# OFA-Sys/ONE-PEACE

Measured on NVIDIA H100. Metric: encoder_samples_per_sec, higher is better.
Workload: dtype bf16

## Files before the change

### one_peace_b200/csrc/gemm_wgmma.cu

```cuda
#include "common.cuh"
#include "gemm.h"

#include <mutex>

namespace opb {

constexpr int kBlockM = 128;
constexpr int kBlockN = 256;
constexpr int kBlockK = 64;
constexpr int kStages = 4;
constexpr int kABytes = kBlockM * kBlockK * 2;
constexpr int kBBytes = kBlockN * kBlockK * 2;
constexpr int kStageBytes = kABytes + kBBytes;
constexpr int kThreads = 384;
constexpr int kBandM = 8;
constexpr int kResidBatch = 16;

struct EpiOperands {
  float2 row[kBlockM];
  float colsum[kBlockN], bias[kBlockN], gamma[kBlockN], colscale[kBlockN];
};
constexpr int kStagerThreads = 96;
constexpr int kSmemBytes = kStages * kStageBytes + 1024 + 2 * sizeof(EpiOperands) + 1024;

struct GemmGeom {
  int M, N, K;
  int kb_inner;
  int num_k_blocks;
  int groups;
  int a_group_c0;
  int b_group_rows;
  int a_mn;
  int b_mn;
  int kb_per_piece;
  int m_pad;
  float* split_ws;
};

OPB_DEVICE void fence_acc(float (&d)[128]) {
#pragma unroll
  for (int i = 0; i < 128; ++i) asm volatile("" : "+f"(d[i])::"memory");
}

template <int TA, int TB>
OPB_DEVICE void wgmma_m64n256k16(float (&d)[128], uint64_t desc_a, uint64_t desc_b, uint32_t scale_d) {
  asm volatile(
      "{\n\t"
      ".reg .pred p;\n\t"
      "setp.ne.b32 p, %130, 0;\n\t"
      "wgmma.mma_async.sync.aligned.m64n256k16.f32.bf16.bf16 "
      "{"
      "%0, %1, %2, %3, %4, %5, %6, %7, %8, %9, %10, %11, %12, %13, %14, %15, "
      "%16, %17, %18, %19, %20, %21, %22, %23, %24, %25, %26, %27, %28, %29, %30, %31, "
      "%32, %33, %34, %35, %36, %37, %38, %39, %40, %41, %42, %43, %44, %45, %46, %47, "
      "%48, %49, %50, %51, %52, %53, %54, %55, %56, %57, %58, %59, %60, %61, %62, %63, "
      "%64, %65, %66, %67, %68, %69, %70, %71, %72, %73, %74, %75, %76, %77, %78, %79, "
      "%80, %81, %82, %83, %84, %85, %86, %87, %88, %89, %90, %91, %92, %93, %94, %95, "
      "%96, %97, %98, %99, %100, %101, %102, %103, %104, %105, %106, %107, %108, %109, %110, %111, "
      "%112, %113, %114, %115, %116, %117, %118, %119, %120, %121, %122, %123, %124, %125, %126, %127"
      "}, %128, %129, p, 1, 1, %131, %132;\n\t"
      "}\n"
      : "+f"(d[0]), "+f"(d[1]), "+f"(d[2]), "+f"(d[3]), "+f"(d[4]), "+f"(d[5]), "+f"(d[6]), "+f"(d[7]),
        "+f"(d[8]), "+f"(d[9]), "+f"(d[10]), "+f"(d[11]), "+f"(d[12]), "+f"(d[13]), "+f"(d[14]), "+f"(d[15]),
        "+f"(d[16]), "+f"(d[17]), "+f"(d[18]), "+f"(d[19]), "+f"(d[20]), "+f"(d[21]), "+f"(d[22]), "+f"(d[23]),
        "+f"(d[24]), "+f"(d[25]), "+f"(d[26]), "+f"(d[27]), "+f"(d[28]), "+f"(d[29]), "+f"(d[30]), "+f"(d[31]),
        "+f"(d[32]), "+f"(d[33]), "+f"(d[34]), "+f"(d[35]), "+f"(d[36]), "+f"(d[37]), "+f"(d[38]), "+f"(d[39]),
        "+f"(d[40]), "+f"(d[41]), "+f"(d[42]), "+f"(d[43]), "+f"(d[44]), "+f"(d[45]), "+f"(d[46]), "+f"(d[47]),
        "+f"(d[48]), "+f"(d[49]), "+f"(d[50]), "+f"(d[51]), "+f"(d[52]), "+f"(d[53]), "+f"(d[54]), "+f"(d[55]),
        "+f"(d[56]), "+f"(d[57]), "+f"(d[58]), "+f"(d[59]), "+f"(d[60]), "+f"(d[61]), "+f"(d[62]), "+f"(d[63]),
        "+f"(d[64]), "+f"(d[65]), "+f"(d[66]), "+f"(d[67]), "+f"(d[68]), "+f"(d[69]), "+f"(d[70]), "+f"(d[71]),
        "+f"(d[72]), "+f"(d[73]), "+f"(d[74]), "+f"(d[75]), "+f"(d[76]), "+f"(d[77]), "+f"(d[78]), "+f"(d[79]),
        "+f"(d[80]), "+f"(d[81]), "+f"(d[82]), "+f"(d[83]), "+f"(d[84]), "+f"(d[85]), "+f"(d[86]), "+f"(d[87]),
        "+f"(d[88]), "+f"(d[89]), "+f"(d[90]), "+f"(d[91]), "+f"(d[92]), "+f"(d[93]), "+f"(d[94]), "+f"(d[95]),
        "+f"(d[96]), "+f"(d[97]), "+f"(d[98]), "+f"(d[99]), "+f"(d[100]), "+f"(d[101]), "+f"(d[102]), "+f"(d[103]),
        "+f"(d[104]), "+f"(d[105]), "+f"(d[106]), "+f"(d[107]), "+f"(d[108]), "+f"(d[109]), "+f"(d[110]), "+f"(d[111]),
        "+f"(d[112]), "+f"(d[113]), "+f"(d[114]), "+f"(d[115]), "+f"(d[116]), "+f"(d[117]), "+f"(d[118]), "+f"(d[119]),
        "+f"(d[120]), "+f"(d[121]), "+f"(d[122]), "+f"(d[123]), "+f"(d[124]), "+f"(d[125]), "+f"(d[126]), "+f"(d[127])
      : "l"(desc_a), "l"(desc_b), "r"(scale_d), "n"(TA), "n"(TB));
}

template <bool kFusedVar = false>
OPB_DEVICE void load_ln_stats(const GemmEpilogue& ep, int row, int M, float& mu, float& rs) {
  mu = 0.f; rs = 1.f;
  const int rc = row < M ? row : M - 1;
  if (ep.ln_partial != nullptr) {
    float s1 = 0.f, s2 = 0.f;
#pragma unroll 8
    for (int p = 0; p < ep.ln_parts; ++p) {
      const float2 v = *reinterpret_cast<const float2*>(ep.ln_partial + (static_cast<long>(p) * M + rc) * 2);
      s1 += v.x; s2 += v.y;
    }
    mu = s1 / ep.ln_dim;
    const float ex2 = s2 / ep.ln_dim;
    const float var = kFusedVar ? fmaf(-mu, mu, ex2) : __fsub_rn(ex2, __fmul_rn(mu, mu));
    rs = rsqrtf(fmaxf(var, 0.f) + ep.ln_eps);
  } else if (ep.ln_mu != nullptr) {
    mu = ep.ln_mu[rc];
    rs = ep.ln_rstd[rc];
  }
}

OPB_DEVICE float2 ldf2(const float* p) { return *reinterpret_cast<const float2*>(p); }
OPB_DEVICE float quad_sum(float v) {
  v += __shfl_xor_sync(0xffffffffu, v, 1);
  return v + __shfl_xor_sync(0xffffffffu, v, 2);
}

template <int TA, int TB>
OPB_DEVICE void mainloop(float (&d)[128], uint8_t* smem, uint64_t* full, uint64_t* empty, int num_k_blocks, int cw,
                         uint32_t it0) {
  constexpr uint32_t step_a = TA ? 2048 : 32, step_b = TB ? 2048 : 32;
  const bool signal = (threadIdx.x & 31) == 0;
  for (int kb = 0; kb < num_k_blocks; ++kb) {
    const uint32_t it = it0 + kb;
    const uint32_t s = it % kStages;
    mbar_wait_quiet(&full[s], (it / kStages) & 1);
    const uint32_t sa = smem_u32(smem + s * kStageBytes) + cw * 8192;
    const uint32_t sb = smem_u32(smem + s * kStageBytes + kABytes);
    fence_acc(d);
    wgmma_fence();
#pragma unroll
    for (int k = 0; k < kBlockK / 16; ++k)
      wgmma_m64n256k16<TA, TB>(d, wgmma_desc_sw128(sa + k * step_a, 8192), wgmma_desc_sw128(sb + k * step_b, 8192),
                               (kb > 0 || k > 0) ? 1u : 0u);
    wgmma_commit();
    fence_acc(d);
    if (kb > 0) {
      wgmma_wait<1>();
      fence_acc(d);
      __syncwarp();
      if (signal) mbar_arrive(&empty[(it - 1) % kStages]);
    }
  }
  wgmma_wait<0>();
  fence_acc(d);
  __syncwarp();
  if (signal) mbar_arrive(&empty[(it0 + num_k_blocks - 1) % kStages]);
}

constexpr bool epi_staged(int epi) { return epi != EPI_LSE_PARTIAL && epi != EPI_SOFTMAX_GRAD; }

template <int EPI>
OPB_DEVICE void stage_epi_operands(EpiOperands* st, const GemmEpilogue& ep, const GemmGeom& geo, int m_blk, int n_blk, int grp,
                                   int t) {
  if (ep.ln_partial != nullptr || ep.ln_mu != nullptr) {
    for (int r = t; r < kBlockM; r += kStagerThreads) {
      float mu, rs;
      load_ln_stats<EPI == EPI_GEGLU_BF16 || EPI == EPI_RESID_F32>(ep, m_blk * kBlockM + r, geo.M, mu, rs);
      st->row[r] = make_float2(mu, rs);
    }
  }
  for (int c = t; c < kBlockN; c += kStagerThreads) {
    const int tc = n_blk * kBlockN + c;
    const bool ok = tc < geo.N;
    const int col = grp * geo.N + tc;
    st->colsum[c] = ok && ep.ln_colsum != nullptr ? ep.ln_colsum[col] : 0.f;
    st->bias[c] = ok && ep.bias != nullptr ? ep.bias[col] : 0.f;
    st->gamma[c] = ok && ep.gamma != nullptr ? ep.gamma[col] : 0.f;
    st->colscale[c] = ok && ep.colscale != nullptr ? ep.colscale[col] : 0.f;
  }
}

template <int EPI>
OPB_DEVICE void epilogue(const float (&d)[128], const GemmEpilogue& ep, const GemmGeom& geo, const EpiOperands* st, int m_blk,
                         int n_blk, int grp, int cw) {
  const int M = geo.M, N = geo.N;
  const int t = threadIdx.x & 127;
  const int lane = t & 31;
  const int quad = lane & 3;
  const int rloc = cw * 64 + (t >> 5) * 16 + (lane >> 2);
  const int rbase = m_blk * kBlockM + rloc;
  const int col0 = n_blk * kBlockN;
  const int gcol0 = grp * N;
#pragma unroll
  for (int h = 0; h < 2; ++h) {
    const int row = rbase + 8 * h;
    bool row_ok = row < M;
    if (ep.out_group > 0 && ep.out_group_valid > 0 && (row % ep.out_group) >= ep.out_group_valid) row_ok = false;
    long out_row = row;
    if (ep.out_group > 0) out_row = static_cast<long>(row / ep.out_group) * ep.out_group_stride + (row % ep.out_group) + ep.out_row_offset;
    long res_row = out_row;
    if (ep.resid_period > 0) res_row = (row % ep.resid_period) + ep.resid_row_offset;

    if constexpr (EPI == EPI_LSE_PARTIAL) {
      const float scale = *ep.scale_ptr;
      const int tgt = row + ep.target_offset;
      const int nv = ep.n_valid > 0 ? ep.n_valid : N;
      float m = -INFINITY;
#pragma unroll
      for (int j = 0; j < 32; ++j) {
        const int col = col0 + 8 * j + 2 * quad;
        if (col < nv) m = fmaxf(m, scale * d[4 * j + 2 * h]);
        if (col + 1 < nv) m = fmaxf(m, scale * d[4 * j + 2 * h + 1]);
      }
      float ssum = 0.f, zsum = 0.f, best = -INFINITY, ztgt = 0.f;
      int best_idx = 0, has_tgt = 0;
#pragma unroll
      for (int j = 0; j < 32; ++j) {
#pragma unroll
        for (int e = 0; e < 2; ++e) {
          const int col = col0 + 8 * j + 2 * quad + e;
          if (col < nv) {
            const float z = scale * d[4 * j + 2 * h + e];
            ssum += __expf(z - m);
            zsum += z;
            if (z > best) { best = z; best_idx = col; }
            if (col == tgt) { ztgt = z; has_tgt = 1; }
          }
        }
      }
#pragma unroll
      for (int o = 1; o <= 2; o <<= 1) {
        const float m2 = __shfl_xor_sync(0xffffffffu, m, o), s2 = __shfl_xor_sync(0xffffffffu, ssum, o);
        const float zs2 = __shfl_xor_sync(0xffffffffu, zsum, o), b2 = __shfl_xor_sync(0xffffffffu, best, o);
        const int i2 = __shfl_xor_sync(0xffffffffu, best_idx, o), h2 = __shfl_xor_sync(0xffffffffu, has_tgt, o);
        const float zt2 = __shfl_xor_sync(0xffffffffu, ztgt, o);
        const float mn = fmaxf(m, m2);
        ssum = (m > -INFINITY ? ssum * __expf(m - mn) : 0.f) + (m2 > -INFINITY ? s2 * __expf(m2 - mn) : 0.f);
        m = mn;
        zsum += zs2;
        if (b2 > best || (b2 == best && i2 < best_idx)) { best = b2; best_idx = i2; }
        if (h2) { ztgt = zt2; has_tgt = 1; }
      }
      if (row_ok && quad == 0) {
        float* w = ep.ws + (static_cast<long>(n_blk) * M + row) * 8;
        *reinterpret_cast<float4*>(w) = make_float4(m, ssum, zsum, best);
        *reinterpret_cast<float4*>(w + 4) = make_float4(__int_as_float(best_idx), ztgt, has_tgt ? 1.f : 0.f, 0.f);
      }
    } else if constexpr (EPI == EPI_SOFTMAX_GRAD) {
      const float scale = *ep.scale_ptr;
      const float gscale = scale * ep.coef;
      const int tgt = row + ep.target_offset;
      const float lse = row_ok ? ep.row_lse[row] : 0.f;
      const float hit = 1.f - ep.eps - ep.eps_i;
      const int nv = ep.n_valid > 0 ? ep.n_valid : N;
      float gz = 0.f;
#pragma unroll
      for (int j = 0; j < 32; ++j) {
        const int col = col0 + 8 * j + 2 * quad;
        if (!row_ok || col >= N) continue;
        float gq[2];
#pragma unroll
        for (int e = 0; e < 2; ++e) {
          const float z = scale * d[4 * j + 2 * h + e];
          float g = __expf(z - lse) - ep.eps_i;
          if (col + e == tgt) g -= hit;
          if (col + e >= nv) g = 0.f;
          gz += g * z;
          gq[e] = g * gscale;
        }
        *reinterpret_cast<uint32_t*>(reinterpret_cast<__nv_bfloat16*>(ep.out) + out_row * ep.ldo + col) = pack_bf16x2(gq[0], gq[1]);
      }
      gz = quad_sum(gz);
      if (row_ok && quad == 0) ep.ws[static_cast<long>(n_blk) * M + row] = gz;
    } else {
      const float2 mr = (ep.ln_partial != nullptr || ep.ln_mu != nullptr) ? st->row[rloc + 8 * h] : make_float2(0.f, 1.f);
      const float mu = mr.x, rs = mr.y;
      const bool has_ln = ep.ln_colsum != nullptr;
      float st_sum = 0.f, st_sq = 0.f;
      if constexpr (EPI == EPI_GEGLU_BF16) {
        __nv_bfloat16* out = reinterpret_cast<__nv_bfloat16*>(ep.out) + out_row * ep.ldo + n_blk * (kBlockN / 2);
#pragma unroll
        for (int j = 0; j < 16; ++j) {
          const int tc = 8 * j + 2 * quad;
          float g0 = d[4 * j + 2 * h], g1 = d[4 * j + 2 * h + 1];
          float l0 = d[4 * (j + 16) + 2 * h], l1 = d[4 * (j + 16) + 2 * h + 1];
          if (has_ln) {
            const float2 cg = ldf2(st->colsum + tc), cl = ldf2(st->colsum + tc + kBlockN / 2);
            g0 = rs * (g0 - mu * cg.x); g1 = rs * (g1 - mu * cg.y);
            l0 = rs * (l0 - mu * cl.x); l1 = rs * (l1 - mu * cl.y);
          }
          if (ep.bias != nullptr) {
            const float2 bg = ldf2(st->bias + tc), bl = ldf2(st->bias + tc + kBlockN / 2);
            g0 += bg.x; g1 += bg.y; l0 += bl.x; l1 += bl.y;
          }
          const float u0 = gelu_erf(g0) * l0, u1 = gelu_erf(g1) * l1;
          st_sum += u0 + u1;
          st_sq += u0 * u0 + u1 * u1;
          if (row_ok) *reinterpret_cast<uint32_t*>(out + tc) = pack_bf16x2(u0, u1);
        }
        st_sum = quad_sum(st_sum);
        st_sq = quad_sum(st_sq);
        if (row_ok && quad == 0 && ep.stats_out != nullptr) {
          *reinterpret_cast<float2*>(ep.stats_out + (static_cast<long>(n_blk * 2) * M + row) * 2) = make_float2(st_sum, st_sq);
          *reinterpret_cast<float2*>(ep.stats_out + (static_cast<long>(n_blk * 2 + 1) * M + row) * 2) = make_float2(0.f, 0.f);
        }
      } else {
#pragma unroll
        for (int jb = 0; jb < 32; jb += kResidBatch) {
          float2 res[kResidBatch];
          if constexpr (EPI == EPI_RESID_F32) {
            if (ep.resid != nullptr && row_ok) {
              const float* rp = ep.resid + res_row * ep.ldr + gcol0;
#pragma unroll
              for (int jj = 0; jj < kResidBatch; ++jj) {
                const int tc = col0 + 8 * (jb + jj) + 2 * quad;
                if (tc < N) res[jj] = ldf2(rp + tc);
              }
            }
          }
#pragma unroll
          for (int jj = 0; jj < kResidBatch; ++jj) {
            const int j = jb + jj;
            const int lc = 8 * j + 2 * quad;
            const int tc = col0 + lc;
            if (tc >= N) continue;
            const int col = gcol0 + tc;
            float x0 = d[4 * j + 2 * h], x1 = d[4 * j + 2 * h + 1];
            if (has_ln) {
              const float2 c = ldf2(st->colsum + lc);
              x0 = rs * (x0 - mu * c.x); x1 = rs * (x1 - mu * c.y);
            }
            if (ep.bias != nullptr) {
              const float2 b = ldf2(st->bias + lc);
              x0 += b.x; x1 += b.y;
            }
            if constexpr (EPI == EPI_STORE_BF16 || EPI == EPI_GELU_BF16) {
              if (ep.colscale != nullptr) {
                const float2 s = ldf2(st->colscale + lc);
                x0 *= s.x; x1 *= s.y;
              }
              if constexpr (EPI == EPI_GELU_BF16) { x0 = gelu_erf(x0); x1 = gelu_erf(x1); }
              if (row_ok) *reinterpret_cast<uint32_t*>(reinterpret_cast<__nv_bfloat16*>(ep.out) + out_row * ep.ldo + col) = pack_bf16x2(x0, x1);
            } else {
              if constexpr (EPI == EPI_RESID_F32) {
                if (ep.gamma != nullptr) {
                  const float2 g = ldf2(st->gamma + lc);
                  x0 *= g.x; x1 *= g.y;
                }
                if (ep.resid != nullptr && row_ok) {
                  x0 += res[jj].x; x1 += res[jj].y;
                }
                st_sum += x0 + x1;
                st_sq += x0 * x0 + x1 * x1;
                if (row_ok && ep.out_bf16 != nullptr)
                  *reinterpret_cast<uint32_t*>(reinterpret_cast<__nv_bfloat16*>(ep.out_bf16) + out_row * ep.ldo_bf16 + col) = pack_bf16x2(x0, x1);
              }
              if (row_ok) *reinterpret_cast<float2*>(reinterpret_cast<float*>(ep.out) + out_row * ep.ldo + col) = make_float2(x0, x1);
            }
          }
        }
        if constexpr (EPI == EPI_RESID_F32) {
          st_sum = quad_sum(st_sum);
          st_sq = quad_sum(st_sq);
          if (row_ok && quad == 0 && ep.stats_out != nullptr)
            *reinterpret_cast<float2*>(ep.stats_out + (static_cast<long>(n_blk) * M + row) * 2) = make_float2(st_sum, st_sq);
        }
      }
    }
  }
}

struct TileCoord {
  int piece, grp, m_blk, n_blk;
};
OPB_DEVICE TileCoord tile_coord(int unit, int num_m_tiles, int num_n_tiles, int groups) {
  const int per_group = num_m_tiles * num_n_tiles;
  TileCoord c;
  c.piece = unit / (per_group * groups);
  const int tile = unit - c.piece * per_group * groups;
  c.grp = tile / per_group;
  const int tin = tile - c.grp * per_group;
  const int band = tin / (kBandM * num_n_tiles);
  const int m0 = band * kBandM;
  const int band_rows = min(kBandM, num_m_tiles - m0);
  const int r = tin - m0 * num_n_tiles;
  c.m_blk = m0 + r % band_rows;
  c.n_blk = r / band_rows;
  return c;
}

template <int EPI>
__global__ void __launch_bounds__(kThreads, 1)
gemm_bf16_kernel(const __grid_constant__ CUtensorMap tm_a, const __grid_constant__ CUtensorMap tm_b, const GemmEpilogue ep,
                 const GemmGeom geo) {
  extern __shared__ __align__(1024) uint8_t smem_raw[];
  uint8_t* smem = smem_raw;
  if ((smem_u32(smem) & 1023u) != 0) __trap();
  uint64_t* full = reinterpret_cast<uint64_t*>(smem + kStages * kStageBytes);
  uint64_t* empty = full + kStages;
  uint64_t* epi_full = empty + kStages;
  uint64_t* epi_empty = epi_full + 2;
  EpiOperands* epi_ops = reinterpret_cast<EpiOperands*>(smem + kStages * kStageBytes + 1024);

  const int wg = threadIdx.x >> 7;
  const int num_m_tiles = (geo.M + kBlockM - 1) / kBlockM;
  const int num_n_tiles = (geo.N + kBlockN - 1) / kBlockN;
  const int pieces = geo.kb_per_piece > 0 ? (geo.num_k_blocks + geo.kb_per_piece - 1) / geo.kb_per_piece : 1;
  const int units = num_m_tiles * num_n_tiles * geo.groups * pieces;
  const bool staged = epi_staged(EPI) && geo.kb_per_piece == 0;

  if (threadIdx.x == 0) {
    tma_prefetch_desc(&tm_a);
    tma_prefetch_desc(&tm_b);
    for (int i = 0; i < kStages; ++i) {
      mbar_init(&full[i], 1);
      mbar_init(&empty[i], 8);
    }
    for (int i = 0; i < 2; ++i) {
      mbar_init(&epi_full[i], kStagerThreads);
      mbar_init(&epi_empty[i], 8);
    }
    fence_barrier_init();
  }
  __syncthreads();

  if (wg == 0) {
    asm volatile("setmaxnreg.dec.sync.aligned.u32 40;");
    if (threadIdx.x == 0) {
      uint32_t it = 0;
      for (int unit = blockIdx.x; unit < units; unit += gridDim.x) {
        const TileCoord tc = tile_coord(unit, num_m_tiles, num_n_tiles, geo.groups);
        const int kb0 = geo.kb_per_piece > 0 ? tc.piece * geo.kb_per_piece : 0;
        const int kb1 = geo.kb_per_piece > 0 ? min(geo.num_k_blocks, kb0 + geo.kb_per_piece) : geo.num_k_blocks;
        const int a_row = tc.m_blk * kBlockM;
        const int b_row = tc.grp * geo.b_group_rows + tc.n_blk * kBlockN;
        const int a_c0 = tc.grp * geo.a_group_c0;
        int kin = kb0 % geo.kb_inner, tap = kb0 / geo.kb_inner;
        for (int kb = kb0; kb < kb1; ++kb, ++it) {
          const uint32_t s = it % kStages;
          mbar_wait_quiet(&empty[s], ((it / kStages) & 1) ^ 1);
          uint8_t* sa = smem + s * kStageBytes;
          uint8_t* sb = sa + kABytes;
          mbar_arrive_expect_tx(&full[s], kStageBytes);
          if (geo.a_mn) {
#pragma unroll
            for (int i = 0; i < kBlockM / 64; ++i) tma_load_2d(&tm_a, &full[s], sa + i * 8192, a_row + 64 * i, kb * kBlockK);
          } else {
            tma_load_3d(&tm_a, &full[s], sa, a_c0 + kin * kBlockK, tap, a_row);
          }
          if (geo.b_mn) {
#pragma unroll
            for (int i = 0; i < kBlockN / 64; ++i) tma_load_2d(&tm_b, &full[s], sb + i * 8192, b_row + 64 * i, kb * kBlockK);
          } else {
            tma_load_2d(&tm_b, &full[s], sb, kb * kBlockK, b_row);
          }
          if (++kin == geo.kb_inner) { kin = 0; ++tap; }
        }
      }
    } else if (threadIdx.x >= 32 && staged) {
      uint32_t j = 0;
      for (int unit = blockIdx.x; unit < units; unit += gridDim.x, ++j) {
        const TileCoord tc = tile_coord(unit, num_m_tiles, num_n_tiles, geo.groups);
        mbar_wait_quiet(&epi_empty[j & 1], ((j >> 1) & 1) ^ 1);
        stage_epi_operands<EPI>(&epi_ops[j & 1], ep, geo, tc.m_blk, tc.n_blk, tc.grp, threadIdx.x - 32);
        mbar_arrive(&epi_full[j & 1]);
      }
    }
  } else {
    asm volatile("setmaxnreg.inc.sync.aligned.u32 232;");
    const int cw = wg - 1;
    float d[128];
#pragma unroll
    for (int i = 0; i < 128; ++i) d[i] = 0.f;
    uint32_t it = 0, j = 0;
    for (int unit = blockIdx.x; unit < units; unit += gridDim.x, ++j) {
      const TileCoord tc = tile_coord(unit, num_m_tiles, num_n_tiles, geo.groups);
      const int kb0 = geo.kb_per_piece > 0 ? tc.piece * geo.kb_per_piece : 0;
      const int kb1 = geo.kb_per_piece > 0 ? min(geo.num_k_blocks, kb0 + geo.kb_per_piece) : geo.num_k_blocks;
      if (geo.a_mn) {
        if (geo.b_mn) mainloop<1, 1>(d, smem, full, empty, kb1 - kb0, cw, it);
        else mainloop<1, 0>(d, smem, full, empty, kb1 - kb0, cw, it);
      } else {
        if (geo.b_mn) mainloop<0, 1>(d, smem, full, empty, kb1 - kb0, cw, it);
        else mainloop<0, 0>(d, smem, full, empty, kb1 - kb0, cw, it);
      }
      it += kb1 - kb0;
      if (geo.kb_per_piece > 0) {
        const int t = threadIdx.x & 127, lane = t & 31;
        const int r0 = tc.m_blk * kBlockM + cw * 64 + (t >> 5) * 16 + (lane >> 2);
        float* w = geo.split_ws + static_cast<long>(tc.piece) * geo.m_pad * geo.N;
#pragma unroll
        for (int h = 0; h < 2; ++h) {
#pragma unroll
          for (int c = 0; c < 32; ++c) {
            const int col = tc.n_blk * kBlockN + 8 * c + 2 * (lane & 3);
            if (col < geo.N)
              *reinterpret_cast<float2*>(w + static_cast<long>(r0 + 8 * h) * geo.N + col) = make_float2(d[4 * c + 2 * h], d[4 * c + 2 * h + 1]);
          }
        }
      } else if (staged) {
        mbar_wait_quiet(&epi_full[j & 1], (j >> 1) & 1);
        epilogue<EPI>(d, ep, geo, &epi_ops[j & 1], tc.m_blk, tc.n_blk, tc.grp, cw);
        __syncwarp();
        if ((threadIdx.x & 31) == 0) mbar_arrive(&epi_empty[j & 1]);
      } else {
        epilogue<EPI>(d, ep, geo, nullptr, tc.m_blk, tc.n_blk, tc.grp, cw);
      }
    }
  }
}

__global__ void __launch_bounds__(256)
gemm_split_epilogue_kernel(const GemmEpilogue ep, const GemmGeom geo, int pieces, int epi) {
  __shared__ float red[2][8];
  const int M = geo.M, N = geo.N;
  const int row = blockIdx.x;
  float mu, rs;
  if (ep.ln_partial != nullptr) {
    float s1 = 0.f, s2 = 0.f;
    for (int p = threadIdx.x; p < ep.ln_parts; p += blockDim.x) {
      const float2 v = *reinterpret_cast<const float2*>(ep.ln_partial + (static_cast<long>(p) * M + row) * 2);
      s1 += v.x; s2 += v.y;
    }
    s1 = warp_sum(s1); s2 = warp_sum(s2);
    if ((threadIdx.x & 31) == 0) { red[0][threadIdx.x >> 5] = s1; red[1][threadIdx.x >> 5] = s2; }
    __syncthreads();
    s1 = s2 = 0.f;
    for (int i = 0; i < 8; ++i) { s1 += red[0][i]; s2 += red[1][i]; }
    mu = s1 / ep.ln_dim;
    rs = rsqrtf(fmaxf(s2 / ep.ln_dim - mu * mu, 0.f) + ep.ln_eps);
  } else {
    load_ln_stats(ep, row, M, mu, rs);
  }
  const int t = blockIdx.y;
  const int col = t * kBlockN + threadIdx.x;
  const long slab = static_cast<long>(geo.m_pad) * N;
  float x = 0.f;
  if (col < N) {
    const float* w = geo.split_ws + static_cast<long>(row) * N + col;
    for (int p = 0; p < pieces; ++p) x += w[p * slab];
    if (ep.ln_colsum) x = rs * (x - mu * ep.ln_colsum[col]);
    if (ep.bias) x += ep.bias[col];
    if (epi == EPI_STORE_BF16) {
      if (ep.colscale) x *= ep.colscale[col];
      reinterpret_cast<__nv_bfloat16*>(ep.out)[static_cast<long>(row) * ep.ldo + col] = __float2bfloat16(x);
    } else {
      if (ep.gamma) x *= ep.gamma[col];
      if (ep.resid) x += ep.resid[static_cast<long>(row) * ep.ldr + col];
      reinterpret_cast<float*>(ep.out)[static_cast<long>(row) * ep.ldo + col] = x;
      if (ep.out_bf16) reinterpret_cast<__nv_bfloat16*>(ep.out_bf16)[static_cast<long>(row) * ep.ldo_bf16 + col] = __float2bfloat16(x);
    }
  }
  if (ep.stats_out != nullptr) {
    const float s1 = warp_sum(x), s2 = warp_sum(x * x);
    __syncthreads();
    if ((threadIdx.x & 31) == 0) { red[0][threadIdx.x >> 5] = s1; red[1][threadIdx.x >> 5] = s2; }
    __syncthreads();
    if (threadIdx.x == 0) {
      float a = 0.f, b = 0.f;
      for (int i = 0; i < 8; ++i) { a += red[0][i]; b += red[1][i]; }
      *reinterpret_cast<float2*>(ep.stats_out + (static_cast<long>(t) * M + row) * 2) = make_float2(a, b);
    }
  }
}

typedef CUresult (*PFN_encodeTiled)(CUtensorMap*, CUtensorMapDataType, cuuint32_t, void*, const cuuint64_t*,
                                    const cuuint64_t*, const cuuint32_t*, const cuuint32_t*, CUtensorMapInterleave,
                                    CUtensorMapSwizzle, CUtensorMapL2promotion, CUtensorMapFloatOOBfill);

static PFN_encodeTiled get_encode_fn() {
  static PFN_encodeTiled fn = nullptr;
  static std::once_flag once;
  std::call_once(once, [] {
    void* p = nullptr;
    cudaDriverEntryPointQueryResult qres;
    if (cudaGetDriverEntryPoint("cuTensorMapEncodeTiled", &p, cudaEnableDefault, &qres) == cudaSuccess &&
        qres == cudaDriverEntryPointSuccess) {
      fn = reinterpret_cast<PFN_encodeTiled>(p);
    }
  });
  return fn;
}

int make_tmap_bf16_2d(CUtensorMap* out, const void* ptr, uint64_t rows, uint64_t cols, uint64_t ld,
                      uint32_t box_rows) {
  PFN_encodeTiled enc = get_encode_fn();
  if (enc == nullptr) return OPB_ERR_CUDA;
  if ((reinterpret_cast<uintptr_t>(ptr) & 15) != 0 || (ld * 2) % 16 != 0) return OPB_ERR_INVALID;
  cuuint64_t gdim[2] = {cols, rows};
  cuuint64_t gstride[1] = {ld * 2};
  cuuint32_t box[2] = {static_cast<cuuint32_t>(kBlockK), box_rows};
  cuuint32_t estr[2] = {1, 1};
  CUresult r = enc(out, CU_TENSOR_MAP_DATA_TYPE_BFLOAT16, 2, const_cast<void*>(ptr), gdim, gstride, box, estr,
                   CU_TENSOR_MAP_INTERLEAVE_NONE, CU_TENSOR_MAP_SWIZZLE_128B, CU_TENSOR_MAP_L2_PROMOTION_L2_256B,
                   CU_TENSOR_MAP_FLOAT_OOB_FILL_NONE);
  return r == CUDA_SUCCESS ? OPB_OK : OPB_ERR_CUDA;
}

int make_tmap_bf16_3d(CUtensorMap* out, const void* ptr, uint64_t k_inner, uint64_t taps, uint64_t tap_stride,
                      uint64_t rows, uint64_t row_stride, uint32_t box_rows) {
  PFN_encodeTiled enc = get_encode_fn();
  if (enc == nullptr) return OPB_ERR_CUDA;
  if ((reinterpret_cast<uintptr_t>(ptr) & 15) != 0 || (tap_stride * 2) % 16 != 0 || (row_stride * 2) % 16 != 0)
    return OPB_ERR_INVALID;
  cuuint64_t gdim[3] = {k_inner, taps, rows};
  cuuint64_t gstride[2] = {tap_stride * 2, row_stride * 2};
  cuuint32_t box[3] = {static_cast<cuuint32_t>(kBlockK), 1, box_rows};
  cuuint32_t estr[3] = {1, 1, 1};
  CUresult r = enc(out, CU_TENSOR_MAP_DATA_TYPE_BFLOAT16, 3, const_cast<void*>(ptr), gdim, gstride, box, estr,
                   CU_TENSOR_MAP_INTERLEAVE_NONE, CU_TENSOR_MAP_SWIZZLE_128B, CU_TENSOR_MAP_L2_PROMOTION_L2_256B,
                   CU_TENSOR_MAP_FLOAT_OOB_FILL_NONE);
  return r == CUDA_SUCCESS ? OPB_OK : OPB_ERR_CUDA;
}

int make_tmap_bf16_batched(CUtensorMap* out, const void* ptr, uint64_t cols, uint64_t rows, uint64_t ld, uint64_t batches,
                           uint64_t batch_stride, uint32_t box_rows) {
  PFN_encodeTiled enc = get_encode_fn();
  if (enc == nullptr) return OPB_ERR_CUDA;
  if ((reinterpret_cast<uintptr_t>(ptr) & 15) != 0 || (ld * 2) % 16 != 0 || (batch_stride * 2) % 16 != 0)
    return OPB_ERR_INVALID;
  cuuint64_t gdim[3] = {cols, rows, batches};
  cuuint64_t gstride[2] = {ld * 2, batch_stride * 2};
  cuuint32_t box[3] = {static_cast<cuuint32_t>(kBlockK), box_rows, 1};
  cuuint32_t estr[3] = {1, 1, 1};
  CUresult r = enc(out, CU_TENSOR_MAP_DATA_TYPE_BFLOAT16, 3, const_cast<void*>(ptr), gdim, gstride, box, estr,
                   CU_TENSOR_MAP_INTERLEAVE_NONE, CU_TENSOR_MAP_SWIZZLE_128B, CU_TENSOR_MAP_L2_PROMOTION_L2_256B,
                   CU_TENSOR_MAP_FLOAT_OOB_FILL_NONE);
  return r == CUDA_SUCCESS ? OPB_OK : OPB_ERR_CUDA;
}

template <int EPI>
static int launch_gemm(const CUtensorMap& ta, const CUtensorMap& tb, const GemmEpilogue& ep, const GemmGeom& geo,
                       cudaStream_t stream) {
  auto kern = gemm_bf16_kernel<EPI>;
  static int resident = 0;
  if (resident == 0) {
    if (cudaFuncSetAttribute(kern, cudaFuncAttributeMaxDynamicSharedMemorySize, kSmemBytes) != cudaSuccess)
      return OPB_ERR_CUDA;
    int per_sm = 0;
    if (cudaOccupancyMaxActiveBlocksPerMultiprocessor(&per_sm, kern, kThreads, kSmemBytes) != cudaSuccess || per_sm < 1)
      return OPB_ERR_CUDA;
    resident = per_sm * sm_count();
  }
  const int pieces = geo.kb_per_piece > 0 ? (geo.num_k_blocks + geo.kb_per_piece - 1) / geo.kb_per_piece : 1;
  const long units = static_cast<long>((geo.M + kBlockM - 1) / kBlockM) * ((geo.N + kBlockN - 1) / kBlockN) * geo.groups * pieces;
  const unsigned grid = static_cast<unsigned>(units < resident ? units : resident);
  kern<<<grid, kThreads, kSmemBytes, stream>>>(ta, tb, ep, geo);
  return cudaGetLastError() == cudaSuccess ? OPB_OK : OPB_ERR_CUDA;
}

static int dispatch_gemm(int epi, const CUtensorMap& ta, const CUtensorMap& tb, const GemmEpilogue& ep, const GemmGeom& geo,
                         cudaStream_t stream) {
  switch (epi) {
    case EPI_STORE_BF16: return launch_gemm<EPI_STORE_BF16>(ta, tb, ep, geo, stream);
    case EPI_GELU_BF16: return launch_gemm<EPI_GELU_BF16>(ta, tb, ep, geo, stream);
    case EPI_GEGLU_BF16: return launch_gemm<EPI_GEGLU_BF16>(ta, tb, ep, geo, stream);
    case EPI_RESID_F32: return launch_gemm<EPI_RESID_F32>(ta, tb, ep, geo, stream);
    case EPI_STORE_F32: return launch_gemm<EPI_STORE_F32>(ta, tb, ep, geo, stream);
    case EPI_LSE_PARTIAL: return launch_gemm<EPI_LSE_PARTIAL>(ta, tb, ep, geo, stream);
    case EPI_SOFTMAX_GRAD: return launch_gemm<EPI_SOFTMAX_GRAD>(ta, tb, ep, geo, stream);
    default: return OPB_ERR_INVALID;
  }
}

struct ByteSpan {
  const char* begin;
  const char* end;
};
static ByteSpan row_span(const void* p, long lo, long hi, long ld, long cols, int esz) {
  const char* c = static_cast<const char*>(p);
  return {c + lo * ld * esz, c + (hi * ld + cols) * esz};
}
static bool spans_meet(const ByteSpan& a, const ByteSpan& b) { return a.begin < b.end && b.begin < a.end; }

static bool resid_aliasing_ok(const GemmEpilogue& ep, int M, long cols) {
  if (ep.resid == nullptr) return true;
  auto out_row = [&](long m) {
    return ep.out_group > 0 ? (m / ep.out_group) * ep.out_group_stride + m % ep.out_group + ep.out_row_offset : m;
  };
  const long g = ep.out_group > 0 ? ep.out_group : M, last = M - 1, q = last / g;
  const long corners[5] = {0, (g < M ? g : M) - 1, q * g, last, q > 0 ? q * g - 1 : 0};
  long lo = out_row(0), hi = lo;
  for (long m : corners) {
    lo = out_row(m) < lo ? out_row(m) : lo;
    hi = out_row(m) > hi ? out_row(m) : hi;
  }
  long rlo = lo, rhi = hi;
  if (ep.resid_period > 0) {
    rlo = ep.resid_row_offset;
    rhi = rlo + (ep.resid_period < M ? ep.resid_period : M) - 1;
  }
  const ByteSpan res = row_span(ep.resid, rlo, rhi, ep.ldr, cols, 4);
  if (ep.out_bf16 != nullptr && spans_meet(res, row_span(ep.out_bf16, lo, hi, ep.ldo_bf16, cols, 2))) return false;
  if (!spans_meet(res, row_span(ep.out, lo, hi, ep.ldo, cols, 4))) return true;
  return ep.resid == ep.out && ep.ldr == ep.ldo && ep.resid_period == 0;
}

static GemmGeom plain_geom(int M, int N, int K) {
  GemmGeom geo;
  geo.M = M; geo.N = N; geo.K = K;
  geo.num_k_blocks = (K + kBlockK - 1) / kBlockK;
  geo.kb_inner = geo.num_k_blocks;
  geo.groups = 1;
  geo.a_group_c0 = 0;
  geo.b_group_rows = 0;
  geo.a_mn = geo.b_mn = 0;
  geo.kb_per_piece = 0;
  geo.m_pad = 0;
  geo.split_ws = nullptr;
  return geo;
}

int gemm_bf16(const void* A, int lda, const void* B, int ldb, int M, int N, int K, int epi, const GemmEpilogue& ep,
              int cta_group, cudaStream_t stream) {
  if (M <= 0 || N <= 0 || K <= 0) return OPB_ERR_INVALID;
  if (K % 8 != 0 || N % 8 != 0 || lda % 8 != 0 || ldb % 8 != 0) return OPB_ERR_INVALID;
  if (epi == EPI_GEGLU_BF16 && N % kBlockN != 0) return OPB_ERR_INVALID;
  if (cta_group < 0 || cta_group > 2) return OPB_ERR_INVALID;
  if (epi == EPI_RESID_F32 && !resid_aliasing_ok(ep, M, N)) return OPB_ERR_INVALID;
  GemmGeom geo = plain_geom(M, N, K);
  const int m_tiles = (M + kBlockM - 1) / kBlockM, n_tiles = (N + kBlockN - 1) / kBlockN;
  const bool split_ok = (epi == EPI_RESID_F32 || (epi == EPI_STORE_BF16 && ep.stats_out == nullptr)) && ep.workspace != nullptr &&
                        ep.out_group == 0 && ep.resid_period == 0 && M <= 2 * kBlockM && geo.num_k_blocks >= 8;
  int pieces = 1;
  if (split_ok) {
    const long slab_bytes = static_cast<long>(m_tiles) * kBlockM * N * 4;
    pieces = sm_count() / (m_tiles * n_tiles);
    if (pieces > geo.num_k_blocks / 2) pieces = geo.num_k_blocks / 2;
    if (pieces > ep.workspace_bytes / slab_bytes) pieces = static_cast<int>(ep.workspace_bytes / slab_bytes);
    if (pieces >= 2) {
      geo.kb_per_piece = (geo.num_k_blocks + pieces - 1) / pieces;
      pieces = (geo.num_k_blocks + geo.kb_per_piece - 1) / geo.kb_per_piece;
      geo.m_pad = m_tiles * kBlockM;
      geo.split_ws = reinterpret_cast<float*>(ep.workspace);
    }
  }
  CUtensorMap ta, tb;
  int rc = make_tmap_bf16_3d(&ta, A, K, 1, lda, M, lda, kBlockM);
  if (rc != OPB_OK) return rc;
  rc = make_tmap_bf16_2d(&tb, B, N, K, ldb, kBlockN);
  if (rc != OPB_OK) return rc;
  rc = dispatch_gemm(epi, ta, tb, ep, geo, stream);
  if (rc != OPB_OK || geo.kb_per_piece == 0) return rc;
  gemm_split_epilogue_kernel<<<dim3(M, n_tiles), 256, 0, stream>>>(ep, geo, pieces, epi);
  return cudaGetLastError() == cudaSuccess ? OPB_OK : OPB_ERR_CUDA;
}

int gemm_bf16_t(const void* A, int lda, int a_mn, const void* B, int ldb, int b_mn, int M, int N, int K, int epi,
                const GemmEpilogue& ep, int cta_group, cudaStream_t stream) {
  if (M <= 0 || N <= 0 || K <= 0 || lda % 8 != 0 || ldb % 8 != 0 || N % 8 != 0) return OPB_ERR_INVALID;
  if (epi != EPI_STORE_BF16 && epi != EPI_STORE_F32) return OPB_ERR_INVALID;
  if ((!a_mn && K % 8 != 0) || (!b_mn && K % 8 != 0) || (a_mn && M % 8 != 0)) return OPB_ERR_INVALID;
  if (cta_group < 0 || cta_group > 2) return OPB_ERR_INVALID;
  GemmGeom geo = plain_geom(M, N, K);
  geo.a_mn = a_mn ? 1 : 0;
  geo.b_mn = b_mn ? 1 : 0;
  CUtensorMap ta, tb;
  int rc = a_mn ? make_tmap_bf16_2d(&ta, A, K, M, lda, 64) : make_tmap_bf16_3d(&ta, A, K, 1, lda, M, lda, kBlockM);
  if (rc != OPB_OK) return rc;
  rc = b_mn ? make_tmap_bf16_2d(&tb, B, K, N, ldb, 64) : make_tmap_bf16_2d(&tb, B, N, K, ldb, kBlockN);
  if (rc != OPB_OK) return rc;
  return dispatch_gemm(epi, ta, tb, ep, geo, stream);
}

int gemm_bf16_grouped_window(const void* X, const void* W, int rows, int groups, int c_pad, int taps, int n_per_group,
                             int epi, const GemmEpilogue& ep, cudaStream_t stream) {
  if (rows <= 0 || groups <= 0 || taps <= 0 || n_per_group <= 0) return OPB_ERR_INVALID;
  if (c_pad % kBlockK != 0 || n_per_group % 8 != 0 || n_per_group > kBlockN) return OPB_ERR_INVALID;
  if (epi == EPI_GEGLU_BF16 || epi == EPI_LSE_PARTIAL || epi == EPI_SOFTMAX_GRAD) return OPB_ERR_INVALID;
  if (epi == EPI_RESID_F32 && !resid_aliasing_ok(ep, rows, static_cast<long>(groups) * n_per_group)) return OPB_ERR_INVALID;
  GemmGeom geo = plain_geom(rows, n_per_group, taps * c_pad);
  geo.kb_inner = c_pad / kBlockK;
  geo.num_k_blocks = taps * geo.kb_inner;
  geo.groups = groups;
  geo.a_group_c0 = c_pad;
  geo.b_group_rows = n_per_group;
  const long row_stride = static_cast<long>(groups) * c_pad;
  CUtensorMap ta, tb;
  int rc = make_tmap_bf16_3d(&ta, X, row_stride, taps, row_stride, rows, row_stride, kBlockM);
  if (rc != OPB_OK) return rc;
  rc = make_tmap_bf16_2d(&tb, W, static_cast<uint64_t>(groups) * n_per_group, geo.K, geo.K, kBlockN);
  if (rc != OPB_OK) return rc;
  return dispatch_gemm(epi, ta, tb, ep, geo, stream);
}

}
```

Baseline: 756.0.

## Split last partial wave of GEMM tiles across CTAs by consumer half

When the tile count leaves a partial final wave of at most half the grid, each remaining tile becomes two units. In each unit only one consumer warpgroup computes its 64-row half and runs the epilogue, while the other just drains the pipeline barriers. This spreads the tail across more SMs so each one issues half the tensor-core work, shortening the last wave. In exchange, the producer still loads full A and B tiles for both halves, which doubles the tail's memory traffic.

```diff
diff --git a/one_peace_b200/csrc/gemm_wgmma.cu b/one_peace_b200/csrc/gemm_wgmma.cu
--- a/one_peace_b200/csrc/gemm_wgmma.cu
+++ b/one_peace_b200/csrc/gemm_wgmma.cu
@@ -370,6 +370,37 @@
   return c;
 }
 
+struct UnitMap {
+  int whole;
+  int units;
+  OPB_DEVICE int tile(int unit, int& half) const {
+    if (unit < whole) {
+      half = -1;
+      return unit;
+    }
+    half = (unit - whole) & 1;
+    return whole + ((unit - whole) >> 1);
+  }
+};
+OPB_DEVICE UnitMap unit_map(int tiles, int grid, bool split_last_round) {
+  const int whole = tiles - tiles % grid, rem = tiles - whole;
+  UnitMap m{tiles, tiles};
+  if (split_last_round && whole > 0 && rem > 0 && 2 * rem <= grid) {
+    m.whole = whole;
+    m.units = whole + 2 * rem;
+  }
+  return m;
+}
+
+OPB_DEVICE void pass_stages(uint64_t* full, uint64_t* empty, int num_k_blocks, uint32_t it0) {
+  for (int kb = 0; kb < num_k_blocks; ++kb) {
+    const uint32_t it = it0 + kb;
+    mbar_wait_quiet(&full[it % kStages], (it / kStages) & 1);
+    __syncwarp();
+    if ((threadIdx.x & 31) == 0) mbar_arrive(&empty[it % kStages]);
+  }
+}
+
 template <int EPI>
 __global__ void __launch_bounds__(kThreads, 1)
 gemm_bf16_kernel(const __grid_constant__ CUtensorMap tm_a, const __grid_constant__ CUtensorMap tm_b, const GemmEpilogue ep,
@@ -387,7 +418,8 @@
   const int num_m_tiles = (geo.M + kBlockM - 1) / kBlockM;
   const int num_n_tiles = (geo.N + kBlockN - 1) / kBlockN;
   const int pieces = geo.kb_per_piece > 0 ? (geo.num_k_blocks + geo.kb_per_piece - 1) / geo.kb_per_piece : 1;
-  const int units = num_m_tiles * num_n_tiles * geo.groups * pieces;
+  const UnitMap umap = unit_map(num_m_tiles * num_n_tiles * geo.groups * pieces, gridDim.x, geo.kb_per_piece == 0);
+  const int units = umap.units;
   const bool staged = epi_staged(EPI) && geo.kb_per_piece == 0;
 
   if (threadIdx.x == 0) {
@@ -410,7 +442,8 @@
     if (threadIdx.x == 0) {
       uint32_t it = 0;
       for (int unit = blockIdx.x; unit < units; unit += gridDim.x) {
-        const TileCoord tc = tile_coord(unit, num_m_tiles, num_n_tiles, geo.groups);
+        int half;
+        const TileCoord tc = tile_coord(umap.tile(unit, half), num_m_tiles, num_n_tiles, geo.groups);
         const int kb0 = geo.kb_per_piece > 0 ? tc.piece * geo.kb_per_piece : 0;
         const int kb1 = geo.kb_per_piece > 0 ? min(geo.num_k_blocks, kb0 + geo.kb_per_piece) : geo.num_k_blocks;
         const int a_row = tc.m_blk * kBlockM;
@@ -441,7 +474,8 @@
     } else if (threadIdx.x >= 32 && staged) {
       uint32_t j = 0;
       for (int unit = blockIdx.x; unit < units; unit += gridDim.x, ++j) {
-        const TileCoord tc = tile_coord(unit, num_m_tiles, num_n_tiles, geo.groups);
+        int half;
+        const TileCoord tc = tile_coord(umap.tile(unit, half), num_m_tiles, num_n_tiles, geo.groups);
         mbar_wait_quiet(&epi_empty[j & 1], ((j >> 1) & 1) ^ 1);
         stage_epi_operands<EPI>(&epi_ops[j & 1], ep, geo, tc.m_blk, tc.n_blk, tc.grp, threadIdx.x - 32);
         mbar_arrive(&epi_full[j & 1]);
@@ -455,10 +489,14 @@
     for (int i = 0; i < 128; ++i) d[i] = 0.f;
     uint32_t it = 0, j = 0;
     for (int unit = blockIdx.x; unit < units; unit += gridDim.x, ++j) {
-      const TileCoord tc = tile_coord(unit, num_m_tiles, num_n_tiles, geo.groups);
+      int half;
+      const TileCoord tc = tile_coord(umap.tile(unit, half), num_m_tiles, num_n_tiles, geo.groups);
+      const bool idle = half >= 0 && half != cw;
       const int kb0 = geo.kb_per_piece > 0 ? tc.piece * geo.kb_per_piece : 0;
       const int kb1 = geo.kb_per_piece > 0 ? min(geo.num_k_blocks, kb0 + geo.kb_per_piece) : geo.num_k_blocks;
-      if (geo.a_mn) {
+      if (idle) {
+        pass_stages(full, empty, kb1 - kb0, it);
+      } else if (geo.a_mn) {
         if (geo.b_mn) mainloop<1, 1>(d, smem, full, empty, kb1 - kb0, cw, it);
         else mainloop<1, 0>(d, smem, full, empty, kb1 - kb0, cw, it);
       } else {
@@ -481,10 +519,10 @@
         }
       } else if (staged) {
         mbar_wait_quiet(&epi_full[j & 1], (j >> 1) & 1);
-        epilogue<EPI>(d, ep, geo, &epi_ops[j & 1], tc.m_blk, tc.n_blk, tc.grp, cw);
+        if (!idle) epilogue<EPI>(d, ep, geo, &epi_ops[j & 1], tc.m_blk, tc.n_blk, tc.grp, cw);
         __syncwarp();
         if ((threadIdx.x & 31) == 0) mbar_arrive(&epi_empty[j & 1]);
-      } else {
+      } else if (!idle) {
         epilogue<EPI>(d, ep, geo, nullptr, tc.m_blk, tc.n_blk, tc.grp, cw);
       }
     }
```

Result: faster. 770.6 (median of 6 runs) (+1.9%).
